# lambdaclass/AES_zero_knowledge_proof_circuit

Hardware: AMD Instinct MI355X
Metric: AES-ECB blocks proven/sec (Marlin), proof verifies (higher is better)
Workload: dtype u32 limbs (253-bit Fr / 377-bit Fq modular integers)

## Files before the change

### aes_zero_knowledge_proof_circuit_amd/api.py

```python
import ctypes as C
import os

import numpy as np

HERE = os.path.dirname(os.path.abspath(__file__))
CIRCUIT_AES, CIRCUIT_OPS_XOR, CIRCUIT_OPS_ADD = 0, 1, 2
KEY_NO_TABLES = 1
PARITY = "parity"


class ZkAesError(RuntimeError):
    """The Err(..) side of the reference's anyhow::Result."""


def lib_path():
    return os.path.join(HERE, "libzkaes.so")


_lib = None


def lib():
    global _lib
    if _lib is None:
# ... 416 lines not shown

def msm_fold_window_sums_dev(curve_id, dev_ptr, world, n_total):
    out = C.create_string_buffer(96)
    inf = C.c_int()
    _check(lib().zkaes_msm_fold_window_sums_dev(int(curve_id), C.c_void_p(dev_ptr), int(world), C.c_size_t(n_total), out, C.byref(inf)))
    return out.raw, bool(inf.value)


def msm_fold_partials_dev(curve_id, dev_ptr, world):
    out = C.create_string_buffer(96)
    inf = C.c_int()
    _check(lib().zkaes_msm_fold_partials_dev(int(curve_id), C.c_void_p(dev_ptr), int(world), out, C.byref(inf)))
    return out.raw, bool(inf.value)


def msm_table(curve_id, bases_bytes, scalars_bytes, window_bits, srs=False):
    n = len(scalars_bytes) // 32
    out = C.create_string_buffer(96)
    inf = C.c_int()
    if srs:
        if int(curve_id) != 377:
            raise ValueError("the SRS (twisted Edwards) table path exists for BLS12-377 only")
        _check(lib().zkaes_msm_table_srs(bytes(bases_bytes), bytes(scalars_bytes), C.c_size_t(n), int(window_bits), out, C.byref(inf)))
    else:
        _check(lib().zkaes_msm_table(int(curve_id), bytes(bases_bytes), bytes(scalars_bytes), C.c_size_t(n), int(window_bits), out, C.byref(inf)))
    return out.raw, bool(inf.value)


def msm_bench(curve_id, bases_bytes, scalars_bytes, reps=3):
    n = len(scalars_bytes) // 32
    t, a = C.c_double(), C.c_double()
    _check(lib().zkaes_msm_bench(int(curve_id), bytes(bases_bytes), bytes(scalars_bytes), C.c_size_t(n), int(reps), C.byref(t), C.byref(a)))
    return t.value, a.value


def msm_bench_synth(n, window_bits=0, reps=3, want_point=False):
    t, a = C.c_double(), C.c_double()
    out = C.create_string_buffer(96)
    _check(lib().zkaes_msm_bench_synth(C.c_size_t(n), int(window_bits), int(reps), C.byref(t), C.byref(a), out))
# ... 35 lines not shown
```

### aes_zero_knowledge_proof_circuit_amd/csrc/capi_kernels.hip

```cpp
#include "../../include/zkaes.h"
#include <cstring>
#include <string>
#include <vector>
#include "hip_util.hpp"
#include "marlin.hpp"
#include "te28.cuh"
#include <algorithm>
#include <chrono>

typedef unsigned int v4u __attribute__((ext_vector_type(4)));
__global__ void __launch_bounds__(256) k_stream_copy(uint4 *__restrict__ dst_, const uint4 *__restrict__ src_, size_t n16) {
    v4u *dst = (v4u *)dst_; const v4u *src = (const v4u *)src_;
    size_t base = (size_t)blockIdx.x * 1024 + threadIdx.x;
    if (base + 768 < n16) {
        v4u v0 = __builtin_nontemporal_load(src + base), v1 = __builtin_nontemporal_load(src + base + 256);
        v4u v2 = __builtin_nontemporal_load(src + base + 512), v3 = __builtin_nontemporal_load(src + base + 768);
        __builtin_nontemporal_store(v0, dst + base); __builtin_nontemporal_store(v1, dst + base + 256);
        __builtin_nontemporal_store(v2, dst + base + 512); __builtin_nontemporal_store(v3, dst + base + 768);
    } else {
        for (size_t i = base; i < n16; i += 256) dst[i] = src[i];
    }
}


// ... 96 lines not shown
    WorkspaceGuard ws;
    zk::XYZZ<Fq> r = zk::gpu::msm<Curve>(ws, db28, ds, n, s);
    if (reps > 0) {
        zk::gpu::MsmStats before = zk::gpu::msm_stats(false);
        EventGuard e0, e1;
        zk::gpu::event_record(e0, s);
        for (int i = 0; i < reps; i++) r = zk::gpu::msm<Curve>(ws, db28, ds, n, s);
        zk::gpu::event_record(e1, s);
        float ms = zk::gpu::event_elapsed_ms(e0, e1);
        zk::gpu::MsmStats after = zk::gpu::msm_stats(false);
        if (ms_total) *ms_total = ms / reps;
        if (ms_acc) *ms_acc = (after.accumulate_ms - before.accumulate_ms) / reps;
    }
    give_affine(r.to_affine(), out_xy, out_inf);
}
template <class Curve, bool EDWARDS> void run_msm_table(const uint8_t *bases, const uint8_t *scalars, size_t n, int c, uint8_t *out_xy, int *out_inf) {
    using Fq = typename Curve::Fq; using Fr = typename Curve::Fr;
    if (c < 2 || c > 22) throw std::invalid_argument("window bits must be in [2, 22]");
    if (n && (!bases || !scalars)) throw std::invalid_argument("zkaes_msm_table: null argument");
    zk::gpu::require_device();
    const size_t nt = (size_t)zk::gpu::table_windows<Curve>(c);
    if ((uint64_t)nt * n >= (1ull << 30)) throw std::invalid_argument("zkaes_msm_table: n x table copies exceeds the 2^30 base indices of one MSM");
    StreamGuard s;
    DevPtr<zk::Affine<Fq>> tab(nt * n);
    DevPtr<Fr> ds(n);
    zk::gpu::h2d(tab, bases, n * 96, s); zk::gpu::h2d(ds, scalars, n * 32, s);
    zk::gpu::build_window_tables<Curve>(tab, n, c, s);
    WorkspaceGuard ws;
    zk::Affine<Fq> a;
    if constexpr (EDWARDS) {
        DevPtr<zk::Niels28<typename Curve::FqP>> tabte(nt * n);
        zk::gpu::convert_bases_te<Curve>(tabte, tab, nt * n, s);
        a = zk::gpu::msm_table<Curve>(ws, tabte, n, 0, c, ds, n, s).to_affine();
    } else {
        DevPtr<zk::Affine28<typename Curve::FqP>> tab28(nt * n);
        zk::gpu::convert_bases<Curve>(tab28, tab, nt * n, s);
        a = zk::gpu::msm_table<Curve>(ws, tab28, n, 0, c, ds, n, s).to_affine();
    }
    give_affine(a, out_xy, out_inf);
}
template <class Curve> void run_msm_window_sums_dev(const uint8_t *bases, const uint8_t *scalars, size_t n_local, size_t n_total, void *dev_out, size_t dev_out_bytes) {
    using Fq = typename Curve::Fq; using Fr = typename Curve::Fr;
    zk::gpu::require_device();
    int c = 0, nwin = 0;
    zk::gpu::msm_sharded_plan<Curve>(n_total, &c, &nwin);
    if (!dev_out || dev_out_bytes < (size_t)nwin * sizeof(zk::XYZZ<Fq>)) throw std::invalid_argument("zkaes_msm_window_sums_dev: device buffer too small for the window sums");
    if (n_local > n_total) throw std::invalid_argument("zkaes_msm_window_sums_dev: n_local > n_total");
// ... 78 lines not shown
int zkaes_msm_fold_partials_dev(int curve_id, const void *dev_in, int world, uint8_t *out_xy, int *out_inf) {
    return guardk([&] {
        if (!dev_in || world < 1 || world > MAX_FOLD_WORLD) throw std::invalid_argument("zkaes_msm_fold_partials_dev: bad arguments (world must be 1..4096)");
        if (curve_id != 377 && curve_id != 381) throw std::invalid_argument("curve_id must be 377 or 381");
        zk::gpu::require_device();
        StreamGuard s;
        if (curve_id == 377) give_affine(zk::gpu::msm_fold_points_device<zk::Bls377>((const zk::XYZZ<zk::Fq377> *)dev_in, world, s).to_affine(), out_xy, out_inf);
        else give_affine(zk::gpu::msm_fold_points_device<zk::Bls381>((const zk::XYZZ<zk::Fq381> *)dev_in, world, s).to_affine(), out_xy, out_inf);
    });
}
int zkaes_msm_table(int curve_id, const uint8_t *bases, const uint8_t *scalars, size_t n, int window_bits, uint8_t *out_xy, int *out_inf) {
    return guardk([&] { if (curve_id == 381) run_msm_table<zk::Bls381, false>(bases, scalars, n, window_bits, out_xy, out_inf); else if (curve_id == 377) run_msm_table<zk::Bls377, false>(bases, scalars, n, window_bits, out_xy, out_inf); else throw std::invalid_argument("curve_id must be 377 or 381"); });
}
int zkaes_msm_table_srs(const uint8_t *bases, const uint8_t *scalars, size_t n, int window_bits, uint8_t *out_xy, int *out_inf) {
    return guardk([&] { run_msm_table<zk::Bls377, true>(bases, scalars, n, window_bits, out_xy, out_inf); });
}
int zkaes_set_device(int ordinal) { return guardk([&] { HIP_CHECK(hipSetDevice(ordinal)); }); }
int zkaes_ntt(int field_id, uint8_t *data, size_t n, int inverse) {
    return guardk([&] { if (field_id == 381) run_ntt<zk::Fr381>(data, n, inverse, 0, 0); else if (field_id == 377) run_ntt<zk::Fr377>(data, n, inverse, 0, 0); else throw std::invalid_argument("field_id must be 377 or 381"); });
}
int zkaes_ntt_coset(int field_id, uint8_t *data, size_t n, int inverse, int coset_c, int lg_big) {
    return guardk([&] {
        if (coset_c <= 0) throw std::invalid_argument("zkaes_ntt_coset: coset index must be positive");
        if (field_id == 381) run_ntt<zk::Fr381>(data, n, inverse, coset_c, lg_big); else if (field_id == 377) run_ntt<zk::Fr377>(data, n, inverse, coset_c, lg_big); else throw std::invalid_argument("field_id must be 377 or 381");
    });
}
int zkaes_ntt_batch(int field_id, uint8_t *data, size_t n, int count, int inverse, const int *coset_c, int lg_big) {
    return guardk([&] {
        if (field_id == 381) run_ntt_batch<zk::Fr381>(data, n, count, inverse, coset_c, lg_big); else if (field_id == 377) run_ntt_batch<zk::Fr377>(data, n, count, inverse, coset_c, lg_big);
        else throw std::invalid_argument("field_id must be 377 or 381");
// ... 312 lines not shown
```

### aes_zero_knowledge_proof_circuit_amd/csrc/consts32.h

```cpp
#pragma once
#include <stdint.h>
#define FR377_BITS 253
#define FR377_P_INIT {0x00000001u, 0x0a118000u, 0xd0000001u, 0x59aa76feu, 0x5c37b001u, 0x60b44d1eu, 0x9a2ca556u, 0x12ab655eu}
#define FR377_ONE_INIT {0xfffffff3u, 0x7d1c7fffu, 0x6ffffff2u, 0x7257f50fu, 0x512c0feeu, 0x16d81575u, 0x2bbb9a9du, 0x0d4bda32u}
#define FR377_R2_INIT {0xb861857bu, 0x25d577bau, 0x8860591fu, 0xcc2c27b5u, 0xe5dc8593u, 0xa7cc008fu, 0xeff1c939u, 0x011fdae7u}
static const uint32_t FR377_P[8] = {0x00000001u, 0x0a118000u, 0xd0000001u, 0x59aa76feu, 0x5c37b001u, 0x60b44d1eu, 0x9a2ca556u, 0x12ab655eu};
static const uint32_t FR377_ONE[8] = {0xfffffff3u, 0x7d1c7fffu, 0x6ffffff2u, 0x7257f50fu, 0x512c0feeu, 0x16d81575u, 0x2bbb9a9du, 0x0d4bda32u};
static const uint32_t FR377_R2[8] = {0xb861857bu, 0x25d577bau, 0x8860591fu, 0xcc2c27b5u, 0xe5dc8593u, 0xa7cc008fu, 0xeff1c939u, 0x011fdae7u};
static const uint32_t FR377_INV = 0xffffffffu;
#define FR381_BITS 255
#define FR381_P_INIT {0x00000001u, 0xffffffffu, 0xfffe5bfeu, 0x53bda402u, 0x09a1d805u, 0x3339d808u, 0x299d7d48u, 0x73eda753u}
#define FR381_ONE_INIT {0xfffffffeu, 0x00000001u, 0x00034802u, 0x5884b7fau, 0xecbc4ff5u, 0x998c4fefu, 0xacc5056fu, 0x1824b159u}
#define FR381_R2_INIT {0xf3f29c6du, 0xc999e990u, 0x87925c23u, 0x2b6cedcbu, 0x7254398fu, 0x05d31496u, 0x9f59ff11u, 0x0748d9d9u}
static const uint32_t FR381_P[8] = {0x00000001u, 0xffffffffu, 0xfffe5bfeu, 0x53bda402u, 0x09a1d805u, 0x3339d808u, 0x299d7d48u, 0x73eda753u};
static const uint32_t FR381_ONE[8] = {0xfffffffeu, 0x00000001u, 0x00034802u, 0x5884b7fau, 0xecbc4ff5u, 0x998c4fefu, 0xacc5056fu, 0x1824b159u};
static const uint32_t FR381_R2[8] = {0xf3f29c6du, 0xc999e990u, 0x87925c23u, 0x2b6cedcbu, 0x7254398fu, 0x05d31496u, 0x9f59ff11u, 0x0748d9d9u};
static const uint32_t FR381_INV = 0xffffffffu;
#define FQ377_BITS 377
#define FQ377_P_INIT {0x00000001u, 0x8508c000u, 0x30000000u, 0x170b5d44u, 0xba094800u, 0x1ef3622fu, 0x00f5138fu, 0x1a22d9f3u, 0x6ca1493bu, 0xc63b05c0u, 0x17c510eau, 0x01ae3a46u}
#define FQ377_ONE_INIT {0xffffff68u, 0x02cdffffu, 0x7fffffb1u, 0x51409f83u, 0x8a7d3ff2u, 0x9f7db3a9u, 0x6e7c6305u, 0x7b4e97b7u, 0x803c84e8u, 0x4cf495bfu, 0xe2fdf49au, 0x008d6661u}
#define FQ377_R2_INIT {0x9400cd22u, 0xb786686cu, 0xb00431b1u, 0x0329fcaau, 0x62d6b46du, 0x22a5f111u, 0x827dc3acu, 0xbfdf7d03u, 0x41790bf9u, 0x837e92f0u, 0x1e914b88u, 0x006dfccbu}
static const uint32_t FQ377_P[12] = {0x00000001u, 0x8508c000u, 0x30000000u, 0x170b5d44u, 0xba094800u, 0x1ef3622fu, 0x00f5138fu, 0x1a22d9f3u, 0x6ca1493bu, 0xc63b05c0u, 0x17c510eau, 0x01ae3a46u};
static const uint32_t FQ377_ONE[12] = {0xffffff68u, 0x02cdffffu, 0x7fffffb1u, 0x51409f83u, 0x8a7d3ff2u, 0x9f7db3a9u, 0x6e7c6305u, 0x7b4e97b7u, 0x803c84e8u, 0x4cf495bfu, 0xe2fdf49au, 0x008d6661u};
static const uint32_t FQ377_R2[12] = {0x9400cd22u, 0xb786686cu, 0xb00431b1u, 0x0329fcaau, 0x62d6b46du, 0x22a5f111u, 0x827dc3acu, 0xbfdf7d03u, 0x41790bf9u, 0x837e92f0u, 0x1e914b88u, 0x006dfccbu};
// ... 29 lines not shown
static const uint32_t G1_377_COFACTOR[4] = {0x00000000u, 0x00000000u, 0x30000000u, 0x170b5d44u};
#define G2_377_COFACTOR_LIMBS 16
static const uint32_t G2_377_COFACTOR[16] = {0x00000001u, 0x00000000u, 0x90000000u, 0x452217ccu, 0xba094800u, 0xa0f3622fu, 0x6676bd09u, 0xd693e8c3u, 0xfae2e189u, 0x8c505634u, 0xe1dcc40cu, 0xfbb36b00u, 0xa6f6a829u, 0xddd88d99u, 0x8ae9562au, 0x0026ba55u};
static const uint64_t BLS12_377_X = 0x8508c00000000001ULL;
#define BLS12_377_FINAL_EXP_LIMBS 63
static const uint32_t BLS12_377_FINAL_EXP[63] = {0x00000002u, 0x0a118000u, 0xb0000001u, 0xcf664765u, 0xe68b3800u, 0xc242c0cbu, 0x0c71fe44u, 0xa47662d7u, 0x40a4efb0u, 0xffc594c3u, 0xb3ee4dc0u, 0x9d4f7bf7u, 0x22a24f5bu, 0x44805f5au, 0xa89998a8u, 0x2f530533u, 0x224ec7d8u, 0x5d716080u, 0xca519301u, 0x1368df8du, 0x17a058bfu, 0xef0199c1u, 0xe54706e1u, 0x4f168ac9u, 0x2eb34320u, 0x9c8f5a7bu, 0x7d50f353u, 0x7c976b42u, 0x027819b8u, 0xf3d95a3eu, 0xbdae7647u, 0x7fdda393u, 0x60f50b26u, 0xbee2660du, 0xe5546ebfu, 0x82fe2158u, 0x7e9fadc0u, 0xdc712eceu, 0x0db9ec0du, 0x898b8d13u, 0xc2bf75cfu, 0x555a89a4u, 0xac9eb555u, 0xa3f771b0u, 0xf2cfbf1fu, 0x7e79b0b2u, 0xfca5f4ebu, 0x13793762u, 0x04e2a70cu, 0x2ddd28e6u, 0xc8fd5918u, 0x621371f3u, 0x8c5374bau, 0x7f41de8du, 0xff3f31bfu, 0xd2f282b4u, 0x748856b5u, 0x4a82c4feu, 0x66da4c66u, 0x06c94748u, 0xaf4801c5u, 0x41d9d66cu, 0x0134ed81u};
#define FQ377_TE_S_INIT {0xd831a0a2u, 0x6de9ca9au, 0x0eb51c8eu, 0xa8aff422u, 0x93607959u, 0x5a76e6c5u, 0xd3806339u, 0x57f38956u, 0xa0c6fe30u, 0xc50636f4u, 0xf52bfd14u, 0x018f4652u}
#define FQ377_TE_SI_INIT {0x8894e1e4u, 0x3fabdfd0u, 0xcc1f55aau, 0xcbf921ddu, 0x460edc0cu, 0xd17deff1u, 0x7897028du, 0xd394e81eu, 0x0912681au, 0xc29c995du, 0xaff9d568u, 0x01515e6cu}
#define FQ377_TE_F_INIT {0xead605e4u, 0xfb7c0ab8u, 0xe2752c7au, 0x363b93d1u, 0x144be536u, 0xd2246835u, 0x429f2077u, 0xeb8bf6ddu, 0x0234d423u, 0x3a9efda2u, 0xba0c72a4u, 0x013c7943u}
#define FQ377_TE_FI_INIT {0xfd76a6bdu, 0x3b092ce1u, 0xbba32683u, 0x925230d9u, 0xe991a197u, 0x872d5d2fu, 0xa82b2ab0u, 0x8367c527u, 0xef662a15u, 0xe285bbb3u, 0x9283e729u, 0x0160527au}
#define FQ377_TE_K2D_INIT {0x44a706c6u, 0xf24b7e84u, 0x80faa8fau, 0xeae02375u, 0x7ef38fa5u, 0x0f4d7cf2u, 0xc5f2bb26u, 0x5597097du, 0x0d95a93eu, 0x8bf6c1ddu, 0xfbff628au, 0x01784602u}
#define FQ377_TE_SIF_INIT {0xa38cfd11u, 0xface0c97u, 0x0adb8383u, 0x8cc7c229u, 0xd44ae9cbu, 0x4765cd5fu, 0x22354029u, 0x9ae986d8u, 0x252ab9bdu, 0xc3dc7860u, 0xc8942395u, 0x00486011u}
#define FQ377_TE_K2D_28_INIT {0x706c521u, 0xdf4444au, 0x8fa7e68u, 0x371b2aau, 0xdd6cd3du, 0xebe579eu, 0x3577a6au, 0x1d3f1c6u, 0x2ada318u, 0x2a73d9du, 0x7da6ef5u, 0xce09495u, 0xfed4ab8u, 0x0001813u}
#define FQ377_TE_SI_28_INIT {0x4e1e338u, 0x09d0889u, 0x5a9d7bdu, 0x00869f5u, 0xcb9f841u, 0xfcb79bcu, 0x14fcb3bu, 0xd78b460u, 0x9add89fu, 0x66e4a72u, 0xcdeb434u, 0x3157be7u, 0x5ed67e0u, 0x000140eu}
#define FQ377_TE_SIF_28_INIT {0xcfd10d5u, 0x9457a38u, 0x383e475u, 0x7e96cb8u, 0x388e8d9u, 0xd00b5abu, 0xd32ebe1u, 0x0c15e03u, 0x5ac3c51u, 0xa270ad8u, 0xe68d2ebu, 0xbe54908u, 0x8029609u, 0x00001c4u}
static const uint8_t ARK_TEST_RNG_SEED[32] = {1,0,0,0, 23,0,0,0, 200,1,0,0, 210,30,0,0, 0,0,0,0, 0,0,0,0, 0,0,0,0, 0,0,0,0};
```

### aes_zero_knowledge_proof_circuit_amd/csrc/kernels_msm.hip

```cpp
#include <cstring>
#include <rocprim/device/device_radix_sort.hpp>
#include <rocprim/device/device_scan.hpp>
#include <chrono>
#include <cstdio>
#include <cstdlib>
#include <mutex>
#include <vector>
#include "hip_util.hpp"
#include "te28.cuh"

namespace zk {
namespace gpu {

template <class P> struct WeierLaw { using Params = P; using Base = Affine28<P>; using Acc = Acc28<P>; static constexpr bool edwards = false; };
template <class P> struct EdwardsLaw { using Params = P; using Base = Niels28<P>; using Acc = AccTE<P>; static constexpr bool edwards = true; };

static MsmStats g_stats;
static std::mutex g_stats_mu;
MsmStats msm_stats(bool reset) {
    std::lock_guard<std::mutex> g(g_stats_mu);
    MsmStats s = g_stats;
    if (reset) g_stats = MsmStats();
    return s;
}
// ... 207 lines not shown
__global__ void __launch_bounds__(64, 2) k_accumulate(const typename Law::Base *__restrict__ bases, const uint32_t *__restrict__ vals,
                                                       const uint32_t *__restrict__ start, const uint32_t *__restrict__ end, const uint32_t *__restrict__ order,
                                                       uint32_t nbuckets_total, uint32_t cap, typename Law::Acc *__restrict__ buckets,
                                                       uint32_t *__restrict__ deferred, uint32_t deferred_cap, uint32_t *__restrict__ deferred_count) {
    using P = typename Law::Params;
    using G = FpMsm<P>;
    [[maybe_unused]] uint64_t bias = 0;
    if constexpr (Law::edwards) bias = FpMsm<P>::hot_loop_bias();
    uint32_t t = blockIdx.x * blockDim.x + threadIdx.x;
    if (t >= nbuckets_total) return;
    uint32_t k = order[t];
    uint32_t s = start[k], e = end[k];
    if (e - s > cap) e = s + cap;
    if constexpr (Law::edwards) {
        AccTE<P> acc = te_identity<P>();
        if (s < e) {
            uint32_t idx = vals[s];
            Niels28<P> p = niels_load_signed<P>(bases + (idx & VAL_INDEX), idx >> 31);
            for (uint32_t i = s; i < e; i++) {
                const uint32_t cur = idx;
                if (i + 1 < e) idx = vals[i + 1];
                const Niels28<P> *next = bases + (idx & VAL_INDEX);
                if (cur & VAL_SKIP) { p = niels_load_signed<P>(next, idx >> 31); continue; }
                te_madd_hot<P>(acc, p, cur >> 31, next, idx >> 31, bias);
            }
        }
        buckets[k] = acc;
    } else {
        Acc28<P> acc;
        bool acc_inf = true;
        if (s < e) {
            uint32_t idx = vals[s];
            Affine28<P> nxt = bases[idx & VAL_INDEX];
            for (uint32_t i = s; i < e; i++) {
// ... 42 lines not shown
    if (total > max_segments) total = max_segments;
    if constexpr (Law::edwards) { if (nlist == 0) return; }
    if (blockIdx.x * blockDim.x < total) {
        __shared__ A sh[64];
        __shared__ uint32_t key[64];
        uint32_t q = NO_SLOT;
        A acc;
        if (t < total) {
            uint32_t lo = 0, hi = nlist;
            while (hi - lo > 1) { uint32_t mid = (lo + hi) >> 1; if (ovf_off[mid] <= t) lo = mid; else hi = mid; }
            q = lo;
            const uint32_t k = ovf_bucket[q], j = t - ovf_off[q];
            uint32_t s = start[k] + (j + 1) * cap, e = s + cap < end[k] ? s + cap : end[k];
            if constexpr (Law::edwards) {
                acc = te_identity<P>();
                for (uint32_t i = s; i < e; i++) {
                    uint32_t cur = vals[i];
                    if (cur & VAL_SKIP) continue;
                    Niels28<P> p = bases[cur & VAL_INDEX];
                    if (cur >> 31) p = niels_neg<P>(p);
                    te_madd<P>(acc, p);
                }
            } else {
                bool acc_inf = true;
                for (uint32_t i = s; i < e; i++) {
                    uint32_t cur = vals[i];
                    Affine28<P> p = bases[cur & VAL_INDEX];
                    if ((cur & VAL_SKIP) || p.is_inf()) continue;
                    if (cur >> 31) p.y = G::zero().template sub<2>(p.y);
                    if (acc_inf) { acc.x = p.x; acc.y = p.y; acc.zz = G::k_one(); acc.zzz = acc.zz; acc_inf = false; continue; }
                    if (!madd28(acc, p)) {
                        uint32_t slot = atomicAdd(deferred_count, 1u);
                        if (slot < deferred_cap) { deferred[2 * slot] = k; deferred[2 * slot + 1] = cur; }
                    }
                }
// ... 162 lines not shown
        if (quad < half) quad_store<P>(pt + quad * PT_WORDS, q, te_add_quad<P>(quad_load<P>(pt + quad * PT_WORDS, q), quad_load<P>(pt + (quad + half) * PT_WORDS, q), q));
        __syncthreads();
    }
}
template <class P>
__global__ void __launch_bounds__(RQ_THREADS) k_reduce_rc(const AccTE<P> *__restrict__ seg_s, const AccTE<P> *__restrict__ seg_w, int lgR, int lgC, AccTE<P> *__restrict__ out) {
    __shared__ uint32_t pt[RQ_QUADS * PT_WORDS];
    const uint32_t R = 1u << lgR, C = 1u << lgC, jobs = 2 * R + C;
    const uint32_t set = blockIdx.x / jobs, job = blockIdx.x % jobs, quad = threadIdx.x >> 2;
    const int q = threadIdx.x & 3;
    const AccTE<P> *src = (job < R ? seg_w : seg_s) + ((size_t)set << (lgR + lgC));
    uint32_t first, stride, len;
    if (job < 2 * R) { first = (job < R ? job : job - R) << lgC; stride = 1; len = C; }
    else { first = job - 2 * R; stride = C; len = R; }
    FpMsm<P> acc = te_identity_quad<P>(q);
    for (uint32_t i = quad; i < len; i += RQ_QUADS)
        acc = te_add_quad<P>(acc, quad_load<P>(reinterpret_cast<const uint32_t *>(src + first + (size_t)i * stride), q), q);
    quad_store<P>(pt + quad * PT_WORDS, q, acc);
    __syncthreads();
    quad_tree_sum<P>(pt, RQ_QUADS, quad, q);
    if (quad == 0) quad_store<P>(reinterpret_cast<uint32_t *>(out + (size_t)set * jobs + job), q, quad_load<P>(pt, q));
}
ZK_HD int quad_weighted_lc(uint32_t M) { int m = 0; while ((1u << m) < M) m++; return M <= 16 ? m : (m + 1) / 2; }
constexpr int RF_OUT = 6;
constexpr int RT_THREADS = 256, RT_QUADS = RT_THREADS / 4;
constexpr int RT_PLANES = RT_QUADS, RT_IDENT = RT_QUADS + 32, RT_SLOTS = RT_IDENT + 1;
__device__ __forceinline__ uint32_t rt_plane_member(uint32_t b, uint32_t i) {
    const uint32_t lo = i & ((1u << b) - 1), hi = i >> b;
    return (hi << (b + 1)) | (1u << b) | lo;
}
template <class P>
__global__ void __launch_bounds__(RT_THREADS) k_reduce_terms(const AccTE<P> *__restrict__ rc, int lgR, int lgC, AccTE<P> *__restrict__ part, XYZZ<Fp<P>> *__restrict__ out, bool to_host) {
    __shared__ uint32_t pt[RT_SLOTS * PT_WORDS];
    const uint32_t R = 1u << lgR, C = 1u << lgC, jobs = 2 * R + C;
    const uint32_t set = blockIdx.x / RF_OUT, term = blockIdx.x % RF_OUT, quad = threadIdx.x >> 2;
    const int q = threadIdx.x & 3;
    const bool plain = term < 2, second = term & 1;
    const AccTE<P> *src = rc + (size_t)set * jobs + (term == 0 ? 0 : (term == 2 || term == 3) ? 2 * R : R);
    const uint32_t M = (term == 2 || term == 3) ? C : R;
    uint32_t first = 0, stride = 0, count = 0;
    if (plain) { first = quad; stride = RT_QUADS; count = quad < M ? (M - quad + RT_QUADS - 1) / RT_QUADS : 0; }
    else {
        const int lc = quad_weighted_lc(M);
        const uint32_t c1 = 1u << lc, r1 = M >> lc, G = second ? r1 : c1, S = second ? c1 : r1, g = quad >> 2, p = quad & 3;
        if (g < G && p < S) { count = (S - p + 3) / 4; first = second ? g * c1 + p : p * c1 + g; stride = second ? 4 : 4 * c1; }
    }
    FpMsm<P> acc = te_identity_quad<P>(q);
    for (uint32_t i = 0; i < count; i++) acc = te_add_quad<P>(acc, quad_load<P>(reinterpret_cast<const uint32_t *>(src + first + (size_t)i * stride), q), q);
    quad_store<P>(pt + quad * PT_WORDS, q, acc);
    if (quad == 0) quad_store<P>(pt + RT_IDENT * PT_WORDS, q, te_identity_quad<P>(q));
    __syncthreads();
    const int nsteps = plain ? 6 : 11;
    for (int step = 0; step < nsteps; step++) {
        bool active = false;
        uint32_t dst = 0, a = 0, b = 0;
        if (plain) { const uint32_t half = (RT_QUADS / 2) >> step; active = quad < half; dst = a = quad; b = quad + half; }
        else if (step == 0) { active = (quad & 3) < 2; dst = a = quad; b = quad + 2; }
        else if (step == 1) { active = (quad & 3) == 0; dst = a = quad; b = quad + 1; }
        else if (step == 2) { active = quad < 16; const uint32_t pl = quad >> 2, j = quad & 3; dst = RT_PLANES + 8 * pl + j; a = 4 * rt_plane_member(pl, 2 * j); b = 4 * rt_plane_member(pl, 2 * j + 1); }
        else if (step == 3) { active = quad < 8; const uint32_t pl = quad >> 1, j = quad & 1; dst = a = RT_PLANES + 8 * pl + j; b = a + 2; }
        else if (step == 4) { active = quad < 4; dst = a = RT_PLANES + 8 * quad; b = a + 1; }
        else { active = quad == 0; dst = a = RT_PLANES + 24; const int h = step - 5; b = (h & 1) ? RT_PLANES + 8 * (2 - h / 2) : a; }
        if (active) quad_store<P>(pt + dst * PT_WORDS, q, te_add_quad<P>(quad_load<P>(pt + a * PT_WORDS, q), quad_load<P>(pt + b * PT_WORDS, q), q));
// ... 181 lines not shown
    [[maybe_unused]] bool te_host_tail = false;
#ifdef ZKAES_MEASURE
    for (int rep = (knockin() & 2) ? 0 : 1; rep < 2; rep++)
#endif
    {
    if constexpr (Law::edwards)
        hipLaunchKernelGGL((k_reduce_l1_pair<A>), dim3((unsigned)((2 * segs * nsets + 63) / 64)), dim3(64), 0, s, (const A *)S.buckets.p, c, nsets, (A *)S.seg_s.p, (A *)S.seg_w.p);
    else
        hipLaunchKernelGGL((k_reduce_l1<A>), dim3((unsigned)((segs * nsets + 63) / 64)), dim3(64), 0, s, (const A *)S.buckets.p, c, nsets, (A *)S.seg_s.p, (A *)S.seg_w.p);
    HIP_LAUNCH_CHECK();
    if constexpr (Law::edwards) {
        const int lgG = c - 3 > 0 ? c - 3 : 0, lgC = (lgG + 1) / 2, lgR = lgG - lgC;
        if (lgC > 8) throw GpuError("msm: more than 2^19 buckets per set");
        const unsigned jobs = 2u * (1u << lgR) + (1u << lgC);
        A *rc = (A *)S.partial.p, *part = rc + (size_t)nsets * jobs;
        hipLaunchKernelGGL((k_reduce_rc<P>), dim3((unsigned)nsets * jobs), dim3(RQ_THREADS), 0, s, (const A *)S.seg_s.p, (const A *)S.seg_w.p, lgR, lgC, rc);
        HIP_LAUNCH_CHECK();
        te_host_tail = !dev_wsum_out && nsets <= 4;
        hipLaunchKernelGGL((k_reduce_terms<P>), dim3((unsigned)(RF_OUT * nsets)), dim3(RT_THREADS), 0, s, (const A *)rc, lgR, lgC, part, res, te_host_tail);
        HIP_LAUNCH_CHECK();
        if (!te_host_tail) {
            hipLaunchKernelGGL((k_reduce_combine<P>), dim3((unsigned)nsets), dim3(64), 0, s, (const A *)part, lgR, lgC, res, dev_wsum_out);
            HIP_LAUNCH_CHECK();
        }
        te_lgR = lgR; te_lgC = lgC;
    } else {
    hipLaunchKernelGGL((k_reduce_l2<A>), dim3(2u * (unsigned)((groups * nsets + 63) / 64)), dim3(64), 0, s, (const A *)S.seg_s.p, (const A *)S.seg_w.p, c, nsets, (A *)S.partial.p);
    HIP_LAUNCH_CHECK();
    const uint32_t parts = 2 * groups;
    if (nsets == 1 && parts > 2048) {
        uint32_t mid = (parts + 255) / 256;
// ... 681 lines not shown
    while (width > 2 && (uint32_t)(width >> 1) >= hi - lo) width >>= 1;
    for (int s = width >> 1; s > 0; s >>= 1) {
        if ((int)t < s) { A a = sh[t]; PtOps<A>::add(a, sh[t + s]); sh[t] = a; }
        __syncthreads();
    }
    if (t == 0) out[b] = sh[0];
}
template <class P>
__global__ void __launch_bounds__(RQ_THREADS) k_quad_sum(const AccTE<P> *__restrict__ in, uint32_t total, uint32_t per, AccTE<P> *__restrict__ out, uint32_t in_stride, uint32_t out_stride) {
    __shared__ uint32_t pt[RQ_QUADS * PT_WORDS];
    in += (size_t)blockIdx.y * in_stride; out += (size_t)blockIdx.y * out_stride;
    const uint32_t b = blockIdx.x, quad = threadIdx.x >> 2;
    const int q = threadIdx.x & 3;
    const uint32_t lo = b * per, hi = lo + per < total ? lo + per : total;
    FpMsm<P> acc = te_identity_quad<P>(q);
    for (uint32_t i = lo + quad; i < hi; i += RQ_QUADS) acc = te_add_quad<P>(acc, quad_load<P>(reinterpret_cast<const uint32_t *>(in + i), q), q);
    quad_store<P>(pt + quad * PT_WORDS, q, acc);
    __syncthreads();
    quad_tree_sum<P>(pt, RQ_QUADS, quad, q);
    if (quad == 0) quad_store<P>(reinterpret_cast<uint32_t *>(out + b), q, quad_load<P>(pt, q));
}
template <class A>
__global__ void __launch_bounds__(64) k_class_result(const A *__restrict__ in, uint32_t *__restrict__ flags, XYZZ<Fp<typename PtOps<A>::Params>> *__restrict__ out) {
    uint32_t i = threadIdx.x;
    if (i < 2) out[i] = PtOps<A>::to_std(in[i]);
    if (i == 2) { *reinterpret_cast<uint32_t *>(out + 2) = *flags; *flags = 0; }
}

template <class Curve, class Law>
static bool class_sum_impl(MsmWorkspace *ws_, const typename Law::Base *bases, const int8_t *vals, size_t n, XYZZ<typename Curve::Fq> *out, stream_t s_) {
    using A = typename Law::Acc;
// ... 82 lines not shown
```

### aes_zero_knowledge_proof_circuit_amd/csrc/te28.cuh

```cuda
#pragma once
#include "ec28.cuh"

namespace zk {

template <class P>
struct alignas(64) Niels28 { FpMsm<P> ymx, ypx, td; uint32_t pad[6]; };
template <class P>
struct AccTE { FpMsm<P> x, y, z, t; };

struct Te377 {
    using P = Fq377P;
    using G = Fp28<P>;
    using F = Fp<P>;
    ZK_HD static G lit28(const uint32_t (&t)[14]) { G r; for (int i = 0; i < 14; i++) r.l[i] = t[i]; return r; }
    ZK_HD static F lit(const uint32_t (&t)[12]) { F r; for (int i = 0; i < 12; i++) r.l[i] = t[i]; return r; }
    ZK_HD static F s_std() { constexpr uint32_t t[12] = FQ377_TE_S_INIT; return lit(t); }
    ZK_HD static F f_std() { constexpr uint32_t t[12] = FQ377_TE_F_INIT; return lit(t); }
    ZK_HD static F k2d_std() { constexpr uint32_t t[12] = FQ377_TE_K2D_INIT; return lit(t); }
    ZK_HD static G k2d() { constexpr uint32_t t[14] = FQ377_TE_K2D_28_INIT; return lit28(t); }
    ZK_HD static G si() { constexpr uint32_t t[14] = FQ377_TE_SI_28_INIT; return lit28(t); }
    ZK_HD static G sif() { constexpr uint32_t t[14] = FQ377_TE_SIF_28_INIT; return lit28(t); }
};

template <class P>
ZK_HD AccTE<P> te_identity() { AccTE<P> r; r.x = FpMsm<P>::zero(); r.t = r.x; r.y = FpMsm<P>::k_one(); r.z = r.y; return r; }
template <class P>
ZK_HD Niels28<P> niels_identity() { Niels28<P> r; r.ymx = FpMsm<P>::k_one(); r.ypx = r.ymx; r.td = FpMsm<P>::zero(); return r; }
template <class P>
ZK_HD Niels28<P> niels_neg(const Niels28<P> &n) { Niels28<P> r; r.ymx = n.ypx; r.ypx = n.ymx; r.td = FpMsm<P>::zero().template sub<2>(n.td); return r; }

template <class P>
ZK_HD void te_madd(AccTE<P> &a, const Niels28<P> &n) {
    using G = FpMsm<P>;
    G A = a.y.template sub_lazy<3>(a.x) * n.ymx;
    G B = a.y.add_lazy(a.x) * n.ypx;
    G C = a.t * n.td;
// ... 16 lines not shown
    G B = G::mul_biased(a.y.add_lazy(a.x), n.ypx, bias);
    G C = G::mul_biased(a.t, n.td, bias);
#if defined(__HIP_DEVICE_COMPILE__)
    asm volatile("" : "+v"(A.l[G::N - 1]), "+v"(B.l[G::N - 1]), "+v"(C.l[G::N - 1]) : : "memory");
#endif
    n = niels_load_signed<P>(next, next_neg);
#if defined(__HIP_DEVICE_COMPILE__)
    asm volatile("" : "+v"(A.l[0]), "+v"(C.l[0]) : : "memory");
#endif
    G E = B.template sub_lazy<2>(A), H = B.add_lazy(A);
    G D = a.z.dbl_lazy();
    G U = D.template sub_lazy<2>(C), V = D.add_lazy(C), F, Gg;
#pragma unroll
    for (int i = 0; i < G::N; i++) { F.l[i] = neg ? V.l[i] : U.l[i]; Gg.l[i] = neg ? U.l[i] : V.l[i]; }
    a.x = G::mul_biased(E, F, bias); a.y = G::mul_biased(Gg, H, bias); a.t = G::mul_biased(E, H, bias); a.z = G::mul_biased(F, Gg, bias);
}
template <class P>
ZK_HD void te_add_inline(AccTE<P> &a, const AccTE<P> &b) {
    using G = FpMsm<P>;
    G A = a.y.template sub<3>(a.x) * b.y.template sub<3>(b.x);
    G B = (a.y + a.x) * (b.y + b.x);
    G C = (a.t * b.t) * Te377::k2d();
    G D = (a.z * b.z).dbl();
    G E = B.template sub<2>(A), H = B + A;
    G F = D.template sub<2>(C), Gg = D + C;
    a.x = E * F; a.y = Gg * H; a.t = E * H; a.z = F * Gg;
}
template <class P>
ZK_EC_FN void te_add(AccTE<P> &a, const AccTE<P> &b) { te_add_inline<P>(a, b); }
template <class P>
// ... 128 lines not shown
```

### include/zkaes.h

```cpp
#ifndef ZKAES_H
#define ZKAES_H
#include <stddef.h>
#include <stdint.h>
#ifdef __cplusplus
extern "C" {
#endif

typedef struct zkaes_pk zkaes_pk;
typedef struct zkaes_vk zkaes_vk;

const char *zkaes_last_error(void);
void zkaes_bytes_free(uint8_t *p);
void zkaes_pk_free(zkaes_pk *pk);
void zkaes_vk_free(zkaes_vk *vk);
int zkaes_device_count(void);
int zkaes_set_device(int ordinal);

int zkaes_synthesize_keys(size_t plaintext_length, zkaes_pk **pk, zkaes_vk **vk);
int zkaes_encrypt(const uint8_t *message, size_t message_len, const uint8_t secret_key[16], const zkaes_pk *pk, uint8_t **proof, size_t *proof_len);
int zkaes_verify_encryption(const zkaes_vk *vk, const uint8_t *proof, size_t proof_len, const uint8_t *ciphertext, size_t ciphertext_len, int *accepted);
int zkaes_proof_roundtrip(const uint8_t *proof, size_t proof_len, uint8_t **out, size_t *out_len);

#define ZKAES_CIRCUIT_AES 0
#define ZKAES_CIRCUIT_OPS_XOR 1
// ... 58 lines not shown
int zkaes_msm(int curve_id, const uint8_t *bases, const uint8_t *scalars, size_t n, uint8_t *out_xy, int *out_inf);
int zkaes_g1_sum(int curve_id, const uint8_t *points_xy, const int *inf, size_t n, uint8_t *out_xy, int *out_inf);
int zkaes_msm_sharded_plan(int curve_id, size_t n_total, int *window_bits, int *n_windows, size_t *bytes_per_rank);
int zkaes_msm_window_sums_dev(int curve_id, const uint8_t *bases, const uint8_t *scalars, size_t n_local, size_t n_total, void *dev_out, size_t dev_out_bytes);
int zkaes_msm_fold_window_sums_dev(int curve_id, const void *dev_in, int world, size_t n_total, uint8_t *out_xy, int *out_inf);
int zkaes_pk_msm_partial_dev(const zkaes_pk *pk, const uint8_t *scalars, size_t n_local, size_t offset, void *dev_out, size_t dev_out_bytes);
int zkaes_msm_fold_partials_dev(int curve_id, const void *dev_in, int world, uint8_t *out_xy, int *out_inf);
int zkaes_pk_serialize_ark_to_file(const zkaes_pk *pk, const char *path, uint64_t *bytes_written);
int zkaes_pk_serialize_ark_to_file_ex(const zkaes_pk *pk, const char *path, int uncompressed, uint64_t *bytes_written);
int zkaes_pk_tables_built(const zkaes_pk *pk, int *built, uint64_t *table_bytes);
int zkaes_pk_srs_info(const zkaes_pk *pk, uint64_t out[6], double secs[2]);
int zkaes_set_default_contexts(size_t n);
int zkaes_srs_hold(int hold);
int zkaes_msm_table(int curve_id, const uint8_t *bases, const uint8_t *scalars, size_t n, int window_bits, uint8_t *out_xy, int *out_inf);
int zkaes_msm_table_srs(const uint8_t *bases, const uint8_t *scalars, size_t n, int window_bits, uint8_t *out_xy, int *out_inf);
int zkaes_msm_bench(int curve_id, const uint8_t *bases, const uint8_t *scalars, size_t n, int reps, double *ms_total, double *ms_accumulate);
int zkaes_msm_bench_synth(size_t n, int window_bits, int reps, double *ms_total, double *ms_accumulate, uint8_t *out_xy);
int zkaes_stream_copy_bench(size_t bytes, int reps, double *gb_per_s);
int zkaes_int_rate_bench(double seconds, double out[8]);
int zkaes_aes_witness(const zkaes_pk *pk, const uint8_t *message, size_t message_len, const uint8_t secret_key[16], uint8_t *z, size_t z_cap, size_t *z_len);

#ifdef __cplusplus
}
#endif
#endif
```

Measured before the change: 94.79.

## Seed Edwards bucket accumulators from first point and add lane-parallel RC reduction

Bucket and reduction loops now start from the first loaded point, converting a Niels point into an extended accumulator, instead of adding to the identity. This removes one full point addition per bucket and per reduction lane. A new k_reduce_rc_lanes kernel splits each row or column job across 16 lanes with a shuffle tree, and is used only when throughput mode is on. A variant API entry exposes that mode for the SRS table MSM. The conversion relies on new precomputed constants and a bias assumption checked by a static_assert.

```diff
diff --git a/aes_zero_knowledge_proof_circuit_amd/api.py b/aes_zero_knowledge_proof_circuit_amd/api.py
--- a/aes_zero_knowledge_proof_circuit_amd/api.py
+++ b/aes_zero_knowledge_proof_circuit_amd/api.py
@@ -454,15 +454,17 @@
     return out.raw, bool(inf.value)
 
 
-def msm_table(curve_id, bases_bytes, scalars_bytes, window_bits, srs=False):
+def msm_table(curve_id, bases_bytes, scalars_bytes, window_bits, srs=False, throughput_variant=False):
     n = len(scalars_bytes) // 32
     out = C.create_string_buffer(96)
     inf = C.c_int()
     if srs:
         if int(curve_id) != 377:
             raise ValueError("the SRS (twisted Edwards) table path exists for BLS12-377 only")
-        _check(lib().zkaes_msm_table_srs(bytes(bases_bytes), bytes(scalars_bytes), C.c_size_t(n), int(window_bits), out, C.byref(inf)))
+        _check(lib().zkaes_msm_table_srs_variant(bytes(bases_bytes), bytes(scalars_bytes), C.c_size_t(n), int(window_bits), 1 if throughput_variant else 0, out, C.byref(inf)))
     else:
+        if throughput_variant:
+            raise ValueError("the throughput variant exists on the SRS (twisted Edwards) path only")
         _check(lib().zkaes_msm_table(int(curve_id), bytes(bases_bytes), bytes(scalars_bytes), C.c_size_t(n), int(window_bits), out, C.byref(inf)))
     return out.raw, bool(inf.value)
 
diff --git a/aes_zero_knowledge_proof_circuit_amd/csrc/capi_kernels.hip b/aes_zero_knowledge_proof_circuit_amd/csrc/capi_kernels.hip
--- a/aes_zero_knowledge_proof_circuit_amd/csrc/capi_kernels.hip
+++ b/aes_zero_knowledge_proof_circuit_amd/csrc/capi_kernels.hip
@@ -134,7 +134,7 @@
     }
     give_affine(r.to_affine(), out_xy, out_inf);
 }
-template <class Curve, bool EDWARDS> void run_msm_table(const uint8_t *bases, const uint8_t *scalars, size_t n, int c, uint8_t *out_xy, int *out_inf) {
+template <class Curve, bool EDWARDS> void run_msm_table(const uint8_t *bases, const uint8_t *scalars, size_t n, int c, uint8_t *out_xy, int *out_inf, bool throughput_variant = false) {
     using Fq = typename Curve::Fq; using Fr = typename Curve::Fr;
     if (c < 2 || c > 22) throw std::invalid_argument("window bits must be in [2, 22]");
     if (n && (!bases || !scalars)) throw std::invalid_argument("zkaes_msm_table: null argument");
@@ -151,6 +151,7 @@
     if constexpr (EDWARDS) {
         DevPtr<zk::Niels28<typename Curve::FqP>> tabte(nt * n);
         zk::gpu::convert_bases_te<Curve>(tabte, tab, nt * n, s);
+        zk::gpu::ThroughputWaits as_between_overlapping_proofs(throughput_variant);
         a = zk::gpu::msm_table<Curve>(ws, tabte, n, 0, c, ds, n, s).to_affine();
     } else {
         DevPtr<zk::Affine28<typename Curve::FqP>> tab28(nt * n);
@@ -259,6 +260,9 @@
 }
 int zkaes_msm_table_srs(const uint8_t *bases, const uint8_t *scalars, size_t n, int window_bits, uint8_t *out_xy, int *out_inf) {
     return guardk([&] { run_msm_table<zk::Bls377, true>(bases, scalars, n, window_bits, out_xy, out_inf); });
+}
+int zkaes_msm_table_srs_variant(const uint8_t *bases, const uint8_t *scalars, size_t n, int window_bits, int throughput_variant, uint8_t *out_xy, int *out_inf) {
+    return guardk([&] { run_msm_table<zk::Bls377, true>(bases, scalars, n, window_bits, out_xy, out_inf, throughput_variant != 0); });
 }
 int zkaes_set_device(int ordinal) { return guardk([&] { HIP_CHECK(hipSetDevice(ordinal)); }); }
 int zkaes_ntt(int field_id, uint8_t *data, size_t n, int inverse) {
diff --git a/aes_zero_knowledge_proof_circuit_amd/csrc/consts32.h b/aes_zero_knowledge_proof_circuit_amd/csrc/consts32.h
--- a/aes_zero_knowledge_proof_circuit_amd/csrc/consts32.h
+++ b/aes_zero_knowledge_proof_circuit_amd/csrc/consts32.h
@@ -67,4 +67,6 @@
 #define FQ377_TE_K2D_28_INIT {0x706c521u, 0xdf4444au, 0x8fa7e68u, 0x371b2aau, 0xdd6cd3du, 0xebe579eu, 0x3577a6au, 0x1d3f1c6u, 0x2ada318u, 0x2a73d9du, 0x7da6ef5u, 0xce09495u, 0xfed4ab8u, 0x0001813u}
 #define FQ377_TE_SI_28_INIT {0x4e1e338u, 0x09d0889u, 0x5a9d7bdu, 0x00869f5u, 0xcb9f841u, 0xfcb79bcu, 0x14fcb3bu, 0xd78b460u, 0x9add89fu, 0x66e4a72u, 0xcdeb434u, 0x3157be7u, 0x5ed67e0u, 0x000140eu}
 #define FQ377_TE_SIF_28_INIT {0xcfd10d5u, 0x9457a38u, 0x383e475u, 0x7e96cb8u, 0x388e8d9u, 0xd00b5abu, 0xd32ebe1u, 0x0c15e03u, 0x5ac3c51u, 0xa270ad8u, 0xe68d2ebu, 0xbe54908u, 0x8029609u, 0x00001c4u}
+#define FQ377_TE_DI_28_INIT {0xc7448d7u, 0xd9fdddau, 0x72e84acu, 0x7593d2au, 0x51c3a60u, 0xc66f1aeu, 0x9769153u, 0xd87e5d4u, 0x5ca9538u, 0x7670b3cu, 0x49cf899u, 0xca3cb94u, 0xb5300dbu, 0x0001a5eu}
+#define FQ377_TE_NDI_28_INIT {0x38bb72au, 0x2ec2225u, 0x8d17bd8u, 0xe7b05d5u, 0x2e3dcaau, 0x694aee6u, 0x5a8620eu, 0x2876b64u, 0x45844bau, 0x2ad8875u, 0x668c7d3u, 0x46ae0cfu, 0xef316e9u, 0x0000084u}
 static const uint8_t ARK_TEST_RNG_SEED[32] = {1,0,0,0, 23,0,0,0, 200,1,0,0, 210,30,0,0, 0,0,0,0, 0,0,0,0, 0,0,0,0, 0,0,0,0};
diff --git a/aes_zero_knowledge_proof_circuit_amd/csrc/kernels_msm.hip b/aes_zero_knowledge_proof_circuit_amd/csrc/kernels_msm.hip
--- a/aes_zero_knowledge_proof_circuit_amd/csrc/kernels_msm.hip
+++ b/aes_zero_knowledge_proof_circuit_amd/csrc/kernels_msm.hip
@@ -245,10 +245,15 @@
     if (e - s > cap) e = s + cap;
     if constexpr (Law::edwards) {
         AccTE<P> acc = te_identity<P>();
-        if (s < e) {
-            uint32_t idx = vals[s];
+        uint32_t i = s, idx = 0;
+        while (i < e && ((idx = vals[i]) & VAL_SKIP)) i++;
+        if (i < e) {
+            const Niels28<P> first = niels_load_signed<P>(bases + (idx & VAL_INDEX), idx >> 31);
+            const bool first_neg = idx >> 31;
+            if (i + 1 < e) idx = vals[i + 1];
             Niels28<P> p = niels_load_signed<P>(bases + (idx & VAL_INDEX), idx >> 31);
-            for (uint32_t i = s; i < e; i++) {
+            acc = te_from_niels<P>(first, first_neg);
+            for (i++; i < e; i++) {
                 const uint32_t cur = idx;
                 if (i + 1 < e) idx = vals[i + 1];
                 const Niels28<P> *next = bases + (idx & VAL_INDEX);
@@ -321,11 +326,13 @@
             uint32_t s = start[k] + (j + 1) * cap, e = s + cap < end[k] ? s + cap : end[k];
             if constexpr (Law::edwards) {
                 acc = te_identity<P>();
+                bool first = true;
                 for (uint32_t i = s; i < e; i++) {
                     uint32_t cur = vals[i];
                     if (cur & VAL_SKIP) continue;
                     Niels28<P> p = bases[cur & VAL_INDEX];
                     if (cur >> 31) p = niels_neg<P>(p);
+                    if (first) { acc = te_from_niels<P>(p, false); first = false; continue; }
                     te_madd<P>(acc, p);
                 }
             } else {
@@ -518,12 +525,44 @@
     if (job < 2 * R) { first = (job < R ? job : job - R) << lgC; stride = 1; len = C; }
     else { first = job - 2 * R; stride = C; len = R; }
     FpMsm<P> acc = te_identity_quad<P>(q);
-    for (uint32_t i = quad; i < len; i += RQ_QUADS)
+    uint32_t i = quad;
+    if (i < len) { acc = quad_load<P>(reinterpret_cast<const uint32_t *>(src + first + (size_t)i * stride), q); i += RQ_QUADS; }
+    for (; i < len; i += RQ_QUADS)
         acc = te_add_quad<P>(acc, quad_load<P>(reinterpret_cast<const uint32_t *>(src + first + (size_t)i * stride), q), q);
     quad_store<P>(pt + quad * PT_WORDS, q, acc);
     __syncthreads();
     quad_tree_sum<P>(pt, RQ_QUADS, quad, q);
     if (quad == 0) quad_store<P>(reinterpret_cast<uint32_t *>(out + (size_t)set * jobs + job), q, quad_load<P>(pt, q));
+}
+constexpr int RL_LANES = 16;
+template <class P>
+__device__ __forceinline__ AccTE<P> lane_xor(const AccTE<P> &a, int d) {
+    AccTE<P> r;
+#pragma unroll
+    for (int i = 0; i < FpMsm<P>::N; i++) { r.x.l[i] = __shfl_xor(a.x.l[i], d); r.y.l[i] = __shfl_xor(a.y.l[i], d); r.z.l[i] = __shfl_xor(a.z.l[i], d); r.t.l[i] = __shfl_xor(a.t.l[i], d); }
+    return r;
+}
+template <class P>
+__global__ void __launch_bounds__(64) k_reduce_rc_lanes(const AccTE<P> *__restrict__ seg_s, const AccTE<P> *__restrict__ seg_w, int lgR, int lgC, uint32_t nsets, AccTE<P> *__restrict__ out) {
+    const uint32_t R = 1u << lgR, C = 1u << lgC, jobs = 2 * R + C;
+    const uint32_t t = blockIdx.x * blockDim.x + threadIdx.x, grp = t / RL_LANES, part = t % RL_LANES;
+    if (grp >= nsets * jobs) return;
+    const uint32_t set = grp / jobs, job = grp % jobs;
+    const AccTE<P> *src = (job < R ? seg_w : seg_s) + ((size_t)set << (lgR + lgC));
+    uint32_t first, stride, len;
+    if (job < 2 * R) { first = (job < R ? job : job - R) << lgC; stride = 1; len = C; }
+    else { first = job - 2 * R; stride = C; len = R; }
+    const uint32_t chunk = (len + RL_LANES - 1) / RL_LANES, cmax = ((R > C ? R : C) + RL_LANES - 1) / RL_LANES;
+    const uint32_t start = part * chunk, cnt = start < len ? (len - start < chunk ? len - start : chunk) : 0;
+    src += first + (size_t)start * stride;
+    AccTE<P> acc = cnt ? src[0] : te_identity<P>();
+    for (uint32_t step = 1; step < cmax + 4; step++) {
+        AccTE<P> b;
+        if (step >= cmax) b = lane_xor<P>(acc, 1 << (step - cmax));
+        else { if (step >= cnt) continue; b = src[(size_t)step * stride]; }
+        te_add_inline<P>(acc, b);
+    }
+    if (part == 0) out[(size_t)set * jobs + job] = acc;
 }
 ZK_HD int quad_weighted_lc(uint32_t M) { int m = 0; while ((1u << m) < M) m++; return M <= 16 ? m : (m + 1) / 2; }
 constexpr int RF_OUT = 6;
@@ -549,8 +588,8 @@
         const uint32_t c1 = 1u << lc, r1 = M >> lc, G = second ? r1 : c1, S = second ? c1 : r1, g = quad >> 2, p = quad & 3;
         if (g < G && p < S) { count = (S - p + 3) / 4; first = second ? g * c1 + p : p * c1 + g; stride = second ? 4 : 4 * c1; }
     }
-    FpMsm<P> acc = te_identity_quad<P>(q);
-    for (uint32_t i = 0; i < count; i++) acc = te_add_quad<P>(acc, quad_load<P>(reinterpret_cast<const uint32_t *>(src + first + (size_t)i * stride), q), q);
+    FpMsm<P> acc = count ? quad_load<P>(reinterpret_cast<const uint32_t *>(src + first), q) : te_identity_quad<P>(q);
+    for (uint32_t i = 1; i < count; i++) acc = te_add_quad<P>(acc, quad_load<P>(reinterpret_cast<const uint32_t *>(src + first + (size_t)i * stride), q), q);
     quad_store<P>(pt + quad * PT_WORDS, q, acc);
     if (quad == 0) quad_store<P>(pt + RT_IDENT * PT_WORDS, q, te_identity_quad<P>(q));
     __syncthreads();
@@ -762,7 +801,10 @@
         if (lgC > 8) throw GpuError("msm: more than 2^19 buckets per set");
         const unsigned jobs = 2u * (1u << lgR) + (1u << lgC);
         A *rc = (A *)S.partial.p, *part = rc + (size_t)nsets * jobs;
-        hipLaunchKernelGGL((k_reduce_rc<P>), dim3((unsigned)nsets * jobs), dim3(RQ_THREADS), 0, s, (const A *)S.seg_s.p, (const A *)S.seg_w.p, lgR, lgC, rc);
+        if (throughput_mode())
+            hipLaunchKernelGGL((k_reduce_rc_lanes<P>), dim3((unsigned)(((size_t)nsets * jobs * RL_LANES + 63) / 64)), dim3(64), 0, s, (const A *)S.seg_s.p, (const A *)S.seg_w.p, lgR, lgC, (uint32_t)nsets, rc);
+        else
+            hipLaunchKernelGGL((k_reduce_rc<P>), dim3((unsigned)nsets * jobs), dim3(RQ_THREADS), 0, s, (const A *)S.seg_s.p, (const A *)S.seg_w.p, lgR, lgC, rc);
         HIP_LAUNCH_CHECK();
         te_host_tail = !dev_wsum_out && nsets <= 4;
         hipLaunchKernelGGL((k_reduce_terms<P>), dim3((unsigned)(RF_OUT * nsets)), dim3(RT_THREADS), 0, s, (const A *)rc, lgR, lgC, part, res, te_host_tail);
@@ -1474,7 +1516,9 @@
     const int q = threadIdx.x & 3;
     const uint32_t lo = b * per, hi = lo + per < total ? lo + per : total;
     FpMsm<P> acc = te_identity_quad<P>(q);
-    for (uint32_t i = lo + quad; i < hi; i += RQ_QUADS) acc = te_add_quad<P>(acc, quad_load<P>(reinterpret_cast<const uint32_t *>(in + i), q), q);
+    uint32_t i = lo + quad;
+    if (i < hi) { acc = quad_load<P>(reinterpret_cast<const uint32_t *>(in + i), q); i += RQ_QUADS; }
+    for (; i < hi; i += RQ_QUADS) acc = te_add_quad<P>(acc, quad_load<P>(reinterpret_cast<const uint32_t *>(in + i), q), q);
     quad_store<P>(pt + quad * PT_WORDS, q, acc);
     __syncthreads();
     quad_tree_sum<P>(pt, RQ_QUADS, quad, q);
diff --git a/aes_zero_knowledge_proof_circuit_amd/csrc/te28.cuh b/aes_zero_knowledge_proof_circuit_amd/csrc/te28.cuh
--- a/aes_zero_knowledge_proof_circuit_amd/csrc/te28.cuh
+++ b/aes_zero_knowledge_proof_circuit_amd/csrc/te28.cuh
@@ -20,6 +20,8 @@
     ZK_HD static G k2d() { constexpr uint32_t t[14] = FQ377_TE_K2D_28_INIT; return lit28(t); }
     ZK_HD static G si() { constexpr uint32_t t[14] = FQ377_TE_SI_28_INIT; return lit28(t); }
     ZK_HD static G sif() { constexpr uint32_t t[14] = FQ377_TE_SIF_28_INIT; return lit28(t); }
+    ZK_HD static G di() { constexpr uint32_t t[14] = FQ377_TE_DI_28_INIT; return lit28(t); }
+    ZK_HD static G ndi() { constexpr uint32_t t[14] = FQ377_TE_NDI_28_INIT; return lit28(t); }
 };
 
 template <class P>
@@ -66,6 +68,21 @@
 #pragma unroll
     for (int i = 0; i < G::N; i++) { F.l[i] = neg ? V.l[i] : U.l[i]; Gg.l[i] = neg ? U.l[i] : V.l[i]; }
     a.x = G::mul_biased(E, F, bias); a.y = G::mul_biased(Gg, H, bias); a.t = G::mul_biased(E, H, bias); a.z = G::mul_biased(F, Gg, bias);
+}
+template <class P>
+ZK_HD AccTE<P> te_from_niels(const Niels28<P> &n, bool neg) {
+    using G = FpMsm<P>;
+    static_assert(5 * (uint64_t)(G::template kp_limb<2>(G::N - 1) - 1) >= 6 * (uint64_t)(G::mod28(G::N - 1) + 1), "sub<2> of a record below 1.2 p would borrow out of the top limb");
+    const G kp = Te377::di(), kn = Te377::ndi();
+    G k;
+#pragma unroll
+    for (int i = 0; i < G::N; i++) k.l[i] = neg ? kn.l[i] : kp.l[i];
+    AccTE<P> r;
+    r.x = n.ypx.template sub<2>(n.ymx) * G::k_one();
+    r.y = n.ypx + n.ymx;
+    r.z = G::k_one().dbl();
+    r.t = n.td * k;
+    return r;
 }
 template <class P>
 ZK_HD void te_add_inline(AccTE<P> &a, const AccTE<P> &b) {
diff --git a/include/zkaes.h b/include/zkaes.h
--- a/include/zkaes.h
+++ b/include/zkaes.h
@@ -96,6 +96,7 @@
 int zkaes_srs_hold(int hold);
 int zkaes_msm_table(int curve_id, const uint8_t *bases, const uint8_t *scalars, size_t n, int window_bits, uint8_t *out_xy, int *out_inf);
 int zkaes_msm_table_srs(const uint8_t *bases, const uint8_t *scalars, size_t n, int window_bits, uint8_t *out_xy, int *out_inf);
+int zkaes_msm_table_srs_variant(const uint8_t *bases, const uint8_t *scalars, size_t n, int window_bits, int throughput_variant, uint8_t *out_xy, int *out_inf);
 int zkaes_msm_bench(int curve_id, const uint8_t *bases, const uint8_t *scalars, size_t n, int reps, double *ms_total, double *ms_accumulate);
 int zkaes_msm_bench_synth(size_t n, int window_bits, int reps, double *ms_total, double *ms_accumulate, uint8_t *out_xy);
 int zkaes_stream_copy_bench(size_t bytes, int reps, double *gb_per_s);
```

Result: no change. 95.56 (median of 6 runs) (+0.8%).
